# jyjblrd/Low-Cost-Mocap

Measured on AMD Instinct MI355X. Metric: triangulated 3D markers/sec at 8 cams x 16 markers, higher is better.
Workload: dtype f64

## Files before the change

low-cost-mocap_amd/csrc/frame_bb.hip:

```cpp
#include "mocap_device.hpp"
#include "kernels.hpp"
#include <cstdlib>
#include "frame_common.hpp"
#include "bb_fold.hpp"

namespace mocap {

constexpr int kBBThreads = 256;
constexpr int kBBWaves = kBBThreads / 64;
constexpr int kBBRecs = kBBThreads + 64;
constexpr int bb_cw(int C) { return C <= 8 ? 1 : 2; }
constexpr uint32_t bb_rec_bytes(int CW) { return 24u + 8u * (uint32_t)CW; }
constexpr bool bb_group_rows(int CT, int ML, int RL) { return CT > 0 && ML > 0 && RL > 0 && CT * ML < 0xFF && (ML & (ML - 1)) == 0; }

constexpr int bb_wg_per_cu(int RL) { return RL == 48 ? 5 : 4; }
constexpr size_t kBBCacheEntry = 4;
constexpr int kBBLdsSlack = 1024;
struct BBLayout {
  size_t bxy, bxy_nx, cnt_nx, bt, rbound, seedkey, slot_key, claimw, recs, rpk, scr, scr_bytes, goff, gcnt, outslot, boff, bnb, seedgh, slot_g, cnt,
      misc, bpl, nh, hits, act, root_blob, root_cam, nact, bnl, bv, pkbase, seen, bcache, total;
  int ncache;
  __host__ __device__ static size_t al(size_t x, size_t a) { return (x + a - 1) / a * a; }
  __host__ __device__ BBLayout(int C, int M, int R, int CW, int wg_per_cu, bool row_words = false) {
    size_t o = 0;
    auto take = [&](size_t bytes, size_t a) {
      o = al(o, a);
      const size_t at = o;
      o += bytes;
      return at;
    };
    bxy = take(sizeof(float2) * (size_t)C * M, 16);
    bxy_nx = take(sizeof(float2) * (size_t)C * M, 16);
    cnt_nx = take(4 * (size_t)C, 4);
    bt = take(sizeof(double) * 10 * ((size_t)C * M + 1), 16);
    rbound = take(8 * (size_t)R, 8);
    claimw = take(8 * (size_t)C, 8);
    pkbase = take(8 * (size_t)CW * R, 8);
    scr = seedkey = take(8 * (size_t)R, 8);
    slot_key = take(8 * (size_t)kBBWaves * R, 8);
    recs = take(8 * (size_t)kBBRecs, 8);
    rpk = take(8 * (size_t)kBBRecs * CW, 8);
    seedgh = take(4 * (size_t)R, 4);
    slot_g = take(4 * (size_t)kBBWaves * R, 4);
    scr_bytes = o - scr;
    goff = take(4 * (size_t)(R + 1), 4);
    gcnt = take(4 * (size_t)R, 4);
    outslot = take(4 * (size_t)R, 4);
    boff = take(4 * (size_t)(R + 1), 4);
    bnb = take(4 * (size_t)R, 4);
    cnt = take(4 * (size_t)C, 4);
    misc = take(4 * 16, 4);
    bpl = take(2 * (size_t)R, 2);
    seen = take(2 * (size_t)R, 2);
    nh = take((size_t)R * C, row_words ? 8 : 1);
    hits = take((size_t)R * C * M, 1);
    act = take((size_t)R * C, row_words ? 8 : 1);
    root_blob = take((size_t)R, 1);
    root_cam = take((size_t)R, 1);
    nact = take((size_t)R, 1);
    bnl = take((size_t)R, 1);
    bv = take((size_t)R, 1);
    bcache = take(0, 4);
    ncache = 0;
    const size_t per_entry = kBBCacheEntry;
    for (int per_cu = wg_per_cu; per_cu >= 1; per_cu--) {
      const size_t lim = ((size_t)160 * 1024 / per_cu - kBBLdsSlack) / 256 * 256;
      if (lim >= o + per_entry * 64) {
        const size_t n = (lim - o) / per_entry;
        ncache = (int)(n > 1024 ? 1024 : n);
        break;
      }
    }
    o += per_entry * (size_t)ncache;
    total = al(o, 16);
  }
};

static int bb_fixed_slots(int C, int M, int R) {
  const char* e = getenv("MOCAP_BB_FIXED_LAYOUT");
  if (e && e[0] == '0') return 0;
  if (C == 8 && M == 16 && R <= 48) return 48;
  if (C == 8 && M == 16 && R <= 64) return 64;
  return 0;
}
static int frame_bb_root_slots(int C, int M, int R) {
  const int f = bb_fixed_slots(C, M, R);
  return f ? f : R;
}
size_t frame_bb_lds_bytes(int C, int M, int R) { return BBLayout(C, M, frame_bb_root_slots(C, M, R), bb_cw(C), bb_wg_per_cu(bb_fixed_slots(C, M, R)), bb_fixed_slots(C, M, R) != 0).total; }
static size_t frame_bb_lds_bytes_min(int C, int M, int R) {
  const BBLayout L(C, M, frame_bb_root_slots(C, M, R), bb_cw(C), bb_wg_per_cu(bb_fixed_slots(C, M, R)), bb_fixed_slots(C, M, R) != 0);
  return L.total - kBBCacheEntry * (size_t)L.ncache;
}
bool frame_bb_fits(int C, int M, int R) {
  return C >= 2 && C <= 16 && M >= 1 && M <= 64 && R >= 1 && R <= 255 && frame_bb_lds_bytes_min(C, M, R) <= (size_t)128 * 1024;
}

template <int CW, uint32_t NONE = 0xFFu>
struct Packed {
  unsigned long long w[CW];
  __device__ __forceinline__ void clear() {
#pragma unroll
    for (int k = 0; k < CW; k++) w[k] = NONE * 0x0101010101010101ull;
  }
  __device__ __forceinline__ void set(int c, uint32_t idx) {
    if (CW == 1)
      w[0] ^= (unsigned long long)(idx ^ NONE) << (8 * c);
    else
      w[c >> 3] ^= (unsigned long long)(idx ^ NONE) << (8 * (c & 7));
  }
  __device__ __forceinline__ uint32_t get(int c) const {
    return CW == 1 ? (uint32_t)(w[0] >> (8 * c)) & 0xFFu : (uint32_t)(w[c >> 3] >> (8 * (c & 7))) & 0xFFu;
  }
};

template <int CT, bool PERK = false>
struct BBCamTables {
  const double* base;
  static constexpr int C = CT;
  static constexpr int kPq = PERK ? 12 * CT * CT : 12 * CT;
  __device__ __forceinline__ ctab_t pq(size_t off) const { return as_ctab(base + off); }
  __device__ __forceinline__ ctab_t rt(size_t off) const { return as_ctab(base + kPq + off); }
  __device__ __forceinline__ ctab_t k4(size_t off) const { return as_ctab(base + kPq + 12 * CT + off); }
  __device__ __forceinline__ const double* f() const { return base + kPq + 16 * CT; }
};
template <bool PERK>
struct BBCamTables<0, PERK> {
  const double* base;
  int C;
  __device__ __forceinline__ ctab_t pq(size_t off) const { return as_ctab(base + off); }
  __device__ __forceinline__ ctab_t rt(size_t off) const { return as_ctab(base + (PERK ? 12 * C * C : 12 * C) + off); }
  __device__ __forceinline__ ctab_t k4(size_t off) const { return as_ctab(base + (PERK ? 12 * C * C + 12 * C : 24 * C) + off); }
  __device__ __forceinline__ const double* f() const { return base + (PERK ? 12 * C * C + 16 * C : 28 * C); }
};

enum { kPrioEval = 0, kPrioSeed = 1, kPrioPhase = 2, kPrioSerial = 3 };
template <int P>
__device__ __forceinline__ void bb_prio() {
  __builtin_amdgcn_s_setprio(P);
}

__device__ __forceinline__ float f32_round_up(double v) {
  const float f = (float)v;
  const int32_t b = __float_as_int(f);
  return (double)f < v ? __int_as_float(b + ((b >> 31) | 1)) : f;
}

template <bool F32R, int CW, int CT, int ML, int RL, bool PERK = false>
struct BBState {
  static constexpr int T = kBBThreads, W = kBBWaves;
  static constexpr bool ROWS = bb_group_rows(CT, ML, RL);
  static constexpr uint32_t kNone = ROWS ? (uint32_t)(CT * ML) : 0xFFu;
  typedef Packed<CW, kNone> Pk;
  static_assert(!ROWS || (CT == 8 && CW == 1), "a row of nh / act as one word: eight cameras");
  __device__ __forceinline__ unsigned long long row_word64(const uint8_t* rows, int r) const { return ((const unsigned long long*)rows)[r]; }
  __device__ static __forceinline__ uint32_t byte_of(unsigned long long w, uint32_t k) { return (uint32_t)(w >> (8u * k)) & 0xFFu; }
  static constexpr bool PLIST = CT > 0 && ML > 0 && RL > 0 && ML < 32 && CT * ML <= 256 && (ML & (ML - 1)) == 0;
  __device__ __forceinline__ uint32_t gbyte(int c, uint32_t k) const { return ROWS ? (uint32_t)c * (uint32_t)ML + k : k; }
  __device__ __forceinline__ size_t grow(int c, uint32_t b) const { return ROWS ? (size_t)b : (size_t)c * M + b; }
  const FrameArgs& p;
  BBCamTables<CT, PERK> cv;
  const int C_, M, R, RS;
  int tid, lane, wave;
  __device__ __forceinline__ void fresh_tid() {
    int t = tid;
    asm volatile("" : "+v"(t));
    tid = t;
    lane = t & 63;
    wave = t >> 6;
  }
  __device__ __forceinline__ int cn() const { return CT > 0 ? CT : C_; }
  enum { PC_OTHER = 0, PC_PAIRS0, PC_PAIRS1, PC_B1_TABLE, PC_ROW_COPY, PC_PHASE_C, PC_SEED_PASS, PC_SEED_PUSH, PC_EVAL, PC_TEST, PC_PHASE_E, PC_COUNT };
#ifdef MOCAP_BB_PHASE_CLOCKS
  uint32_t pc_last = 0, pc_sum[PC_COUNT] = {};
  template <int PH>
  __device__ __forceinline__ void pc_mark() {
    if (__builtin_amdgcn_readfirstlane((int)threadIdx.x >> 6) == 0) {
      const uint32_t now = (uint32_t)__builtin_readcyclecounter();
      pc_sum[PH] += now - pc_last;
      pc_last = now;
    }
  }
  __device__ __forceinline__ void pc_start() { pc_last = (uint32_t)__builtin_readcyclecounter(); }
  __device__ __forceinline__ void pc_flush() const {
    if (threadIdx.x == 0 && !p.n_frames_dev)
      for (int k = 0; k < PC_COUNT; k++) atomicAdd(&p.status[p.n_frames + k], (int)(pc_sum[k] >> 8));
  }
#else
  template <int PH>
  __device__ __forceinline__ void pc_mark() {}
  __device__ __forceinline__ void pc_start() {}
  __device__ __forceinline__ void pc_flush() const {}
#endif
  double* bt;
  float2 *bxy, *bxy_nx;
  int32_t* cnt_nx;
  unsigned long long *rbound, *seedkey, *slot_key, *claimw, *rpk;
  struct BRec { uint32_t gh, rs; };
  BRec* recs;
  uint32_t *goff, *gcnt, *boff, *bnb, *seedgh, *slot_g;
  int32_t *outslot, *cnt, *misc;
  uint16_t* bpl;
  uint8_t *nh, *hits, *act, *root_blob, *root_cam, *nact, *bnl, *bv;
  float* bcache;
  unsigned long long* pkbase;
  uint16_t* seen;
  int ncache;
  unsigned char* scr;
  size_t scr_bytes;
  static constexpr unsigned long long kInfBits = 0x7ff0000000000000ull;

  __device__ BBState(const FrameArgs& p_, unsigned char* smem)
      : p(p_), C_(p_.cv.C), M(ML > 0 ? ML : p_.M), R(p_.K_max), RS(RL > 0 ? RL : p_.K_max), tid(threadIdx.x), lane(threadIdx.x & 63), wave(threadIdx.x >> 6) {
    const int C = cn();
    {
      const unsigned long long ta = (unsigned long long)(uintptr_t)p_.cv.Pq;
      uint32_t tlo = (uint32_t)__builtin_amdgcn_readfirstlane((int)(uint32_t)ta);
      uint32_t thi = (uint32_t)__builtin_amdgcn_readfirstlane((int)(uint32_t)(ta >> 32));
      asm volatile("" : "+s"(tlo), "+s"(thi));
      cv.base = (const double*)(uintptr_t)(((unsigned long long)thi << 32) | tlo);
      if constexpr (CT == 0) cv.C = C;
    }
    const BBLayout L(C, M, RS, CW, bb_wg_per_cu(RL), ROWS);
    bt = (double*)(smem + L.bt);
    bxy = (float2*)(smem + L.bxy);
    bxy_nx = (float2*)(smem + L.bxy_nx);
    cnt_nx = (int32_t*)(smem + L.cnt_nx);
    rbound = (unsigned long long*)(smem + L.rbound);
    seedkey = (unsigned long long*)(smem + L.seedkey);
    slot_key = (unsigned long long*)(smem + L.slot_key);
    claimw = (unsigned long long*)(smem + L.claimw);
    recs = (BRec*)(smem + L.recs);
    rpk = (unsigned long long*)(smem + L.rpk);
    goff = (uint32_t*)(smem + L.goff);
    gcnt = (uint32_t*)(smem + L.gcnt);
    outslot = (int32_t*)(smem + L.outslot);
    boff = (uint32_t*)(smem + L.boff);
    bnb = (uint32_t*)(smem + L.bnb);
    seedgh = (uint32_t*)(smem + L.seedgh);
    slot_g = (uint32_t*)(smem + L.slot_g);
    cnt = (int32_t*)(smem + L.cnt);
    misc = (int32_t*)(smem + L.misc);
    bpl = (uint16_t*)(smem + L.bpl);
    nh = (uint8_t*)(smem + L.nh);
    hits = (uint8_t*)(smem + L.hits);
    act = (uint8_t*)(smem + L.act);
    root_blob = (uint8_t*)(smem + L.root_blob);
    root_cam = (uint8_t*)(smem + L.root_cam);
    nact = (uint8_t*)(smem + L.nact);
    bnl = (uint8_t*)(smem + L.bnl);
    bv = (uint8_t*)(smem + L.bv);
    scr = smem + L.scr;
    scr_bytes = L.scr_bytes;
    bcache = (float*)(smem + L.bcache);
    pkbase = (unsigned long long*)(smem + L.pkbase);
    seen = (uint16_t*)(smem + L.seen);
    ncache = L.ncache;
  }

  struct Line { double a, b, c, den, rden; };
  __device__ __forceinline__ Line epiline(int r, int i) const { return epiline_of(root_cam[r], root_blob[r], i); }
  __device__ __forceinline__ Line epiline_of(int rc, int rb, int i) const {
    const int C = cn();
    const double* Fm = cv.f() + 9 * ((size_t)rc * C + i);
    const float2 rp = bxy[(size_t)rc * M + rb];
    const double x = (double)rp.x, y = (double)rp.y;
    double a = Fm[0] * x + Fm[1] * y + Fm[2];
    double b = Fm[3] * x + Fm[4] * y + Fm[5];
    double c = Fm[6] * x + Fm[7] * y + Fm[8];
    double nu = a * a + b * b;
    nu = nu != 0.0 ? 1.0 / sqrt(nu) : 1.0;
    a *= nu;
    b *= nu;
    c *= nu;
    if (F32R) {
      a = (double)(float)a;
      b = (double)(float)b;
      c = (double)(float)c;
    }
    Line L;
    L.a = a;
    L.b = b;
    L.c = c;
    L.den = sqrt(a * a + b * b);
    L.rden = recip_refined(L.den);
    return L;
  }

  template <bool CHAIN>
  __device__ __forceinline__ unsigned long long match_pairs(const Line& mine, int pair_r, int pair_i, int n_pairs, int gs_shift,
                                                            int cam = 0, int Mi_chain = 0) {
    const int C = cn();
    const int GS = 1 << gs_shift, PPS = 64 >> gs_shift;
    const int k = lane & (GS - 1), q = lane >> gs_shift;
    const int gl0 = lane & ~(GS - 1);
    const unsigned long long gall = gs_shift == 6 ? ~0ull : ((1ull << GS) - 1ull);
    unsigned long long claims = 0ull;
    for (int s0 = 0; s0 < n_pairs; s0 += PPS) {
      const int src = s0 + q;
      const bool has = src < n_pairs;
      const int sl = has ? src : 0;
      const double la = __shfl(mine.a, sl), lb = __shfl(mine.b, sl), lc = __shfl(mine.c, sl);
      const double lden = __shfl(mine.den, sl), lrden = __shfl(mine.rden, sl);
      const int r = __shfl(pair_r, sl);
      const int i = CHAIN ? cam : __shfl(pair_i, sl);
      const int Mi = has ? (CHAIN ? Mi_chain : cnt[i]) : 0;
      const bool valid = k < Mi;
      float2 pt = make_float2(0.f, 0.f);
      double d = 0.0;
      bool hit = false;
      if (valid) {
        pt = bxy[(size_t)i * M + k];
        const double num = fabs(la * (double)pt.x + lb * (double)pt.y + lc);
        d = div_by(num, lden, lrden);
        hit = d < p.gate_px;
      }
      const unsigned long long wm = __ballot(hit);
      const unsigned long long gm = (wm >> gl0) & gall;
      int rank = 0;
      const unsigned int dlo = (unsigned int)__double_as_longlong(d), dhi = (unsigned int)(__double_as_longlong(d) >> 32);
      for (unsigned long long mm = wm; mm;) {
        const int j = __ffsll((long long)mm) - 1;
        mm &= mm - 1;
        const double dj = __longlong_as_double(((long long)__builtin_amdgcn_readlane((int)dhi, j) << 32) |
                                               (unsigned int)__builtin_amdgcn_readlane((int)dlo, j));
        const bool mine_grp = (j & ~(GS - 1)) == gl0 && j != lane;
        rank += (hit && mine_grp && (dj < d || (dj == d && j < lane))) ? 1 : 0;
      }
      if (hit) hits[((size_t)r * C + i) * M + rank] = (uint8_t)gbyte(i, (uint32_t)k);
      const unsigned long long g0 = (__ballot(hit && rank == 0) >> gl0) & gall;
      bool same = false;
      if (valid && g0) {
        const float2 p0 = bxy[(size_t)i * M + (__ffsll((long long)g0) - 1)];
        same = pt.x == p0.x && pt.y == p0.y;
      }
      const unsigned long long cw = __ballot(same);
      if (CHAIN) {
        for (int sh = 0; sh < 64; sh += GS) claims |= (cw >> sh) & gall;
      }
      if (has && k == 0) {
        nh[(size_t)r * C + i] = (uint8_t)__popcll(gm);
        if (!CHAIN) {
          const unsigned long long cm = (cw >> gl0) & gall;
          if (cm) atomicOr(&claimw[i], cm);
        }
      }
    }
    return claims;
  }

  __device__ __forceinline__ void prefetch_lds(int64_t frame) const {
    const int C = cn();
    const float* src = p.blobs + (size_t)frame * C * M * 2;
    const int n_dw = C * M * 2;
    for (int base = wave * 64; base < n_dw; base += T)
      if (base + lane < n_dw)
        __builtin_amdgcn_global_load_lds((const __attribute__((address_space(1))) void*)(src + base + lane),
                                         (__attribute__((address_space(3))) void*)((float*)bxy_nx + base), 4, 0, 0);
    if (wave == 0 && lane < C)
      __builtin_amdgcn_global_load_lds((const __attribute__((address_space(1))) void*)(p.counts + (size_t)frame * C + lane),
                                       (__attribute__((address_space(3))) void*)cnt_nx, 4, 0, 0);
  }
  __device__ __forceinline__ void stage(int64_t frame) {
    fresh_tid();
    const int C = cn();
    float2* t = bxy;
    bxy = bxy_nx;
    bxy_nx = t;
    if (tid < C) {
      const int n = cnt_nx[tid];
      cnt[tid] = n < 0 ? 0 : (n > M ? M : n);
      claimw[tid] = 0ull;
    }
    if (tid == 0) {
      misc[MI_STATUS] = 0;
      misc[MI_OMAX] = 0;
    }
  }

  __device__ void match() {
    fresh_tid();
    const int C = cn();
    __syncthreads();
    int gs_shift = 0;
    while ((1 << gs_shift) < M) gs_shift++;
    const int n0 = cnt[0] < R ? cnt[0] : R;
    {
      for (int r = tid; r < n0; r += T) {
        root_cam[r] = 0;
        root_blob[r] = (uint8_t)r;
      }
      if (tid == 0 && cnt[0] > R) misc[MI_STATUS] |= MOCAP_ST_ROOT_OVERFLOW_;
    }
    __syncthreads();
    auto U_of = [&](int j) {
      const int n = cnt[j];
      return ~claimw[j] & (n >= 64 ? ~0ull : ((1ull << n) - 1ull));
    };
    int n_prov = 0, n_ppairs = 0;
    bool pre = false;
    uint8_t* nh_s = nullptr;
    uint8_t* hits_s = nullptr;
    unsigned long long* pclaim = (unsigned long long*)scr;
    uint8_t* plist = act;
    uint32_t* p_end = goff;
    {
      int Mmax = 0;
      for (int c = 1; c < C; c++) Mmax = cnt[c] > Mmax ? cnt[c] : Mmax;
#pragma nounroll
      for (int stage_ = 0; stage_ < 2; stage_++) {
        const int stage = __builtin_amdgcn_readfirstlane(stage_);
        int NP = n0 * (C - 1);
        if (stage == 1) {
          block_sync_lds();
          pc_mark<PC_PAIRS0>();
          if constexpr (PLIST) {
#pragma unroll
            for (int j = 1; j < CT; j++) {
              const uint32_t U = ~((const uint32_t*)claimw)[2 * j] & ((1u << cnt[j]) - 1u);
              if (lane < ML && ((U >> lane) & 1u)) plist[__builtin_amdgcn_mbcnt_lo(U, (uint32_t)n_prov)] = (uint8_t)(j * ML + lane);
              n_prov += __popc(U);
              n_ppairs += __popc(U) * (CT - 1 - j);
              if (lane == 0) p_end[j] = ((uint32_t)n_ppairs << 16) | (uint32_t)n_prov;
            }
            wave_lds_sync();
          } else
          for (int j = 1; j < C; j++) {
            const int np = __popcll(U_of(j));
            n_prov += np;
            n_ppairs += np * (C - 1 - j);
          }
          pre = n_prov <= 64 && (size_t)n_prov * C * (8 + 1 + (size_t)M) <= scr_bytes;
          if (!pre) break;
          nh_s = (uint8_t*)(pclaim + (size_t)n_prov * C);
          hits_s = nh_s + (size_t)n_prov * C;
          NP = n_ppairs;
        }
        for (int base = wave * 64; base < NP; base += W * 64) {
          const int pi = base + lane;
          const bool have = pi < NP;
          int r = 0, i = 1, Mi = 0;
          Line L = {0, 0, 0, 1, 1};
          if (have) {
            if (stage == 0) {
              r = pi / (C - 1);
              i = 1 + (pi - r * (C - 1));
              L = epiline(r, i);
            } else if constexpr (PLIST) {
              int j = 1;
              uint32_t before = 0;
              const uint32_t key = ((uint32_t)pi << 16) | 0xFFFFu;
              uint32_t pe[CT > 2 ? CT - 2 : 1];
#pragma unroll
              for (int jj = 1; jj <= CT - 2; jj++) pe[jj - 1] = p_end[jj];
#pragma unroll
              for (int jj = 1; jj <= CT - 2; jj++) {
                const bool ge = key >= pe[jj - 1];
                j += ge ? 1 : 0;
                before = ge ? pe[jj - 1] : before;
              }
              const uint32_t acc = before >> 16, pb = before & 0xFFFFu;
              uint32_t ord, off;
              divmod_tiny((uint32_t)pi - acc, (uint32_t)(CT - 1 - j), ord, off);
              r = (int)(pb + ord);
              const int k = plist[r] & (ML - 1);
              i = j + 1 + (int)off;
              L = epiline_of(j, k, i);
            } else {
              int j = 1, acc = 0, pb = 0, span = C - 2;
              unsigned long long U = 0ull;
              for (; j <= C - 2; j++) {
                span = C - 1 - j;
                U = U_of(j);
                const int nj = __popcll(U) * span;
                if (pi < acc + nj) break;
                acc += nj;
                pb += __popcll(U);
              }
              uint32_t ord, off;
              divmod_tiny((uint32_t)(pi - acc), (uint32_t)span, ord, off);
              for (uint32_t t = 0; t < ord; t++) U &= U - 1;
              const int k = __ffsll((long long)U) - 1;
              i = j + 1 + (int)off;
              r = pb + (int)ord;
              L = epiline_of(j, k, i);
            }
            Mi = cnt[i];
          }
          const float2* pts = bxy + (size_t)i * M;
          auto dist = [&](int k) {
            const float2 pt = pts[k];
            return div_by(fabs(L.a * (double)pt.x + L.b * (double)pt.y + L.c), L.den, L.rden);
          };
          unsigned long long hm = 0ull;
          double bd0 = __builtin_huge_val();
          int bk0 = 0;
          if constexpr (ROWS) {
            static_assert(ML % 2 == 0 && ML < 32, "two blobs per word, the slots as bits of one register");
            const float4* pw = (const float4*)pts;
            uint32_t cand = (1u << Mi) - 1u;
            uint32_t hw = 0u;
            if constexpr (F32R) {
              static_assert(CT * ML == 128, "the frame's slots: one word of two blobs per lane");
              uint32_t ob;
              {
                const float4 v = ((const float4*)bxy)[lane];
                const int n = cnt[lane / (ML / 2)], k0 = 2 * (lane % (ML / 2));
                const uint32_t ax = __float_as_uint(v.x) & 0x7FFFFFFFu, ay = __float_as_uint(v.y) & 0x7FFFFFFFu;
                const uint32_t az = __float_as_uint(v.z) & 0x7FFFFFFFu, aw = __float_as_uint(v.w) & 0x7FFFFFFFu;
                const uint32_t m0 = k0 < n ? (ax > ay ? ax : ay) : 0u, m1 = k0 + 1 < n ? (az > aw ? az : aw) : 0u;
                ob = m0 > m1 ? m0 : m1;
                auto up = [](uint32_t x, uint32_t y) { return x > y ? x : y; };
                ob = up(ob, (uint32_t)__builtin_amdgcn_update_dpp(0, (int)ob, 0xB1, 0xf, 0xf, true));
                ob = up(ob, (uint32_t)__builtin_amdgcn_update_dpp(0, (int)ob, 0x4E, 0xf, 0xf, true));
                ob = up(ob, (uint32_t)__builtin_amdgcn_update_dpp(0, (int)ob, 0x141, 0xf, 0xf, true));
                ob = up(ob, (uint32_t)__builtin_amdgcn_update_dpp(0, (int)ob, 0x140, 0xf, 0xf, true));
                const uint32_t r0 = (uint32_t)__builtin_amdgcn_readlane((int)ob, 0), r1 = (uint32_t)__builtin_amdgcn_readlane((int)ob, 16);
                const uint32_t r2 = (uint32_t)__builtin_amdgcn_readlane((int)ob, 32), r3 = (uint32_t)__builtin_amdgcn_readlane((int)ob, 48);
                ob = up(up(r0, r1), up(r2, r3));
                ob = ob < 0x7F800000u ? ob : 0x7F800000u;
              }
              const double om = (double)__uint_as_float(ob);
              const float a32 = (float)L.a, b32 = (float)L.b, c32 = (float)L.c;
              const float thr = f32_round_up(p.gate_px * L.den * (1.0 + 1e-12) + (2.5 * 0x1p-24) * (2.0 * om + fabs(L.c)) * (1.0 + 1e-6));
              uint32_t pm = 0u;
#pragma unroll
              for (int h = ML / 2 - 1; h >= 0; h--) {
                const float4 v = pw[h];
                float t0 = fmaf(a32, v.x, fmaf(b32, v.y, c32)), t1 = fmaf(a32, v.z, fmaf(b32, v.w, c32));
                asm("" : "+v"(t0), "+v"(t1));
                pm = pm + pm + (fabsf(t1) <= thr ? 1u : 0u);
                pm = pm + pm + (fabsf(t0) <= thr ? 1u : 0u);
              }
              cand &= pm;
              while (__ballot(cand != 0u)) {
                if (cand) {
                  const int k = __ffs((int)cand) - 1;
                  cand &= cand - 1u;
                  const double d = dist(k);
                  if (d < p.gate_px) {
                    hw |= 1u << k;
                    if (d < bd0) {
                      bd0 = d;
                      bk0 = k;
                    }
                  }
                }
              }
            } else {
#pragma unroll
              for (int h = 0; h < ML / 2; h++) {
                const float4 v = pw[h];
                const double d0 = div_by(fabs(L.a * (double)v.x + L.b * (double)v.y + L.c), L.den, L.rden);
                const double d1 = div_by(fabs(L.a * (double)v.z + L.b * (double)v.w + L.c), L.den, L.rden);
                const bool h0 = d0 < p.gate_px && ((cand >> (2 * h)) & 1u), h1 = d1 < p.gate_px && ((cand >> (2 * h + 1)) & 1u);
                hw |= h0 ? 1u << (2 * h) : 0u;
                const bool b0 = h0 && d0 < bd0;
                bd0 = b0 ? d0 : bd0;
                bk0 = b0 ? 2 * h : bk0;
                hw |= h1 ? 2u << (2 * h) : 0u;
                const bool b1 = h1 && d1 < bd0;
                bd0 = b1 ? d1 : bd0;
                bk0 = b1 ? 2 * h + 1 : bk0;
              }
            }
            hm = hw;
          } else
#pragma unroll 4
          for (int k = 0; k < Mmax; k++)
            if (k < Mi && dist(k) < p.gate_px) hm |= 1ull << k;
          uint8_t* nhp = stage == 0 ? nh : nh_s;
          uint8_t* hl = (stage == 0 ? hits : hits_s) + ((size_t)r * C + i) * M;
          if (have) nhp[(size_t)r * C + i] = (uint8_t)__popcll(hm);
          unsigned long long rem = hm, claim = 0ull;
          int pos = 0;
          float2 p0 = make_float2(0.f, 0.f);
          if constexpr (ROWS) {
            if (hm) {
              hl[0] = (uint8_t)gbyte(i, (uint32_t)bk0);
              claim = hm;
              if (hm & (hm - 1ull)) {
                claim = 0ull;
                p0 = pts[bk0];
                for (unsigned long long t = hm; t; t &= t - 1) {
                  const int k = __ffsll((long long)t) - 1;
                  const float2 q = pts[k];
                  if (q.x == p0.x && q.y == p0.y) claim |= 1ull << k;
                }
              }
              rem = hm & ~(1ull << bk0);
              pos = 1;
            }
          }
          while (__ballot(rem != 0ull)) {
            if (rem) {
              double bd = __builtin_huge_val();
              int bk = 0;
              if (ROWS && !(rem & (rem - 1ull))) {
                bk = __ffsll((long long)rem) - 1;
              } else
              for (unsigned long long t = rem; t; t &= t - 1) {
                const int k = __ffsll((long long)t) - 1;
                const double d = dist(k);
                if (d < bd) {
                  bd = d;
                  bk = k;
                }
              }
              hl[pos] = (uint8_t)gbyte(i, (uint32_t)bk);
              if (!ROWS && pos == 0) {
                p0 = pts[bk];
                for (unsigned long long t = hm; t; t &= t - 1) {
                  const int k = __ffsll((long long)t) - 1;
                  const float2 q = pts[k];
                  if (q.x == p0.x && q.y == p0.y) claim |= 1ull << k;
                }
              }
              rem &= ~(1ull << bk);
              pos++;
            }
          }
          if (stage == 0) {
            if (claim) atomicOr(&claimw[i], claim);
          } else if (have) {
            pclaim[(size_t)r * C + i] = claim;
          }
        }
      }
    }
    const int NL = M * ((C - 1) * (C - 2) / 2);
    const bool spec = F32R && (size_t)NL * 20 + 8 <= scr_bytes;
    double* sp_den = (double*)scr;
    float* sp_abc = (float*)(sp_den + NL);
    auto sp_base = [&](int j) { return M * ((j - 1) * (C - 1) - (j - 1) * j / 2); };
    if (spec && !pre) {
      int tot = 0;
      for (int j = 1; j <= C - 2; j++) {
        const int n = cnt[j];
        const unsigned long long U = ~claimw[j] & (n >= 64 ? ~0ull : ((1ull << n) - 1ull));
        tot += __popcll(U) * (C - 1 - j);
      }
      for (int l = tid; l < tot; l += T) {
        int j = 1, acc = 0, span = C - 2;
        unsigned long long U = 0ull;
        for (; j <= C - 2; j++) {
          const int n = cnt[j];
          U = ~claimw[j] & (n >= 64 ? ~0ull : ((1ull << n) - 1ull));
          span = C - 1 - j;
          const int nj = __popcll(U) * span;
          if (l < acc + nj) break;
          acc += nj;
        }
        uint32_t ord, off;
        divmod_tiny((uint32_t)(l - acc), (uint32_t)span, ord, off);
        for (uint32_t t = 0; t < ord; t++) U &= U - 1;
        const int k = __ffsll((long long)U) - 1, i = j + 1 + (int)off;
        const int ll = sp_base(j) + k * span + (int)off;
        const Line L = epiline_of(j, k, i);
        sp_den[ll] = L.den;
        sp_abc[3 * ll + 0] = (float)L.a;
        sp_abc[3 * ll + 1] = (float)L.b;
        sp_abc[3 * ll + 2] = (float)L.c;
      }
    }
    __syncthreads();
    pc_mark<PC_PAIRS1>();
    fresh_tid();
    if (wave == 0) bb_prio<kPrioSerial>();
    if (wave == 0 && pre) {
      int jp = 0, kp = 0;
      if constexpr (PLIST) {
        if (lane < n_prov) {
          const int row = plist[lane];
          jp = row / ML;
          kp = row & (ML - 1);
        }
      } else
      if (lane < n_prov) {
        int acc = 0;
        unsigned long long U = 0ull;
        for (jp = 1; jp < C; jp++) {
          U = U_of(jp);
          const int np = __popcll(U);
          if (lane < acc + np) break;
          acc += np;
        }
        for (int t = 0; t < lane - acc; t++) U &= U - 1;
        kp = __ffsll((long long)U) - 1;
      }
      bool real = false;
      for (int i = 1; i < C; i++) {
        wave_lds_sync();
        if (lane < n_prov && jp == i) {
          real = !((claimw[i] >> kp) & 1ull);
          if (real)
            for (int c = i + 1; c < C; c++) {
              const unsigned long long m = pclaim[(size_t)lane * C + c];
              if (m) atomicOr(&claimw[c], m);
            }
        }
      }
      const unsigned long long rm = __ballot(real);
      const int rank = __popcll(rm & ((1ull << lane) - 1ull));
      int n_roots = n0 + __popcll(rm);
      if (real && n0 + rank < R) {
        root_cam[n0 + rank] = (uint8_t)jp;
        root_blob[n0 + rank] = (uint8_t)kp;
        bnl[rank] = (uint8_t)lane;
      }
      if (lane == 0) {
        if (n_roots > R) {
          misc[MI_STATUS] |= MOCAP_ST_ROOT_OVERFLOW_;
          n_roots = R;
        }
        misc[MI_NROOTS] = n_roots;
      }
    } else if (wave == 0) {
      const int cntL = lane < C ? cnt[lane] : 0;
      const unsigned long long clmL = lane < C ? claimw[lane] : 0ull;
      int nr_cam = 0, nr_blob = 0;
      int n_roots = n0;
      bool over = false;
      for (int i = 1; i < C; i++) {
        const int Mi = __builtin_amdgcn_readlane(cntL, i);
        unsigned long long claimed = ((unsigned long long)(unsigned int)__builtin_amdgcn_readlane((int)(clmL >> 32), i) << 32) |
                                     (unsigned int)__builtin_amdgcn_readlane((int)clmL, i);
        const int n_new = n_roots - n0;
        for (int base = 0; base < n_new; base += 64) {
          const int l = base + lane;
          const bool have = l < n_new;
          int j = nr_cam, k = nr_blob;
          if (base) {
            wave_lds_sync();
            j = have ? root_cam[n0 + l] : 0;
            k = have ? root_blob[n0 + l] : 0;
          }
          Line L = {0, 0, 0, 1, 1};
          if (have) {
            if (spec) {
              const int ll = sp_base(j) + k * (C - 1 - j) + (i - j - 1);
              L.a = (double)sp_abc[3 * ll + 0];
              L.b = (double)sp_abc[3 * ll + 1];
              L.c = (double)sp_abc[3 * ll + 2];
              L.den = sp_den[ll];
              L.rden = recip_refined(L.den);
            } else {
              L = epiline_of(j, k, i);
            }
          }
          claimed |= match_pairs<true>(L, n0 + l, i, (n_new - base < 64) ? n_new - base : 64, gs_shift, i, Mi);
        }
        const bool flag = lane < Mi && !((claimed >> lane) & 1ull);
        const unsigned long long mask = __ballot(flag);
        const int pos = __popcll(mask & ((1ull << lane) - 1ull));
        if (flag) {
          const int rr = n_roots + pos;
          if (rr < R) {
            root_cam[rr] = (uint8_t)i;
            root_blob[rr] = (uint8_t)lane;
          }
        }
        int slot = n_new;
        for (unsigned long long mm = mask; mm; slot++) {
          const int jb = __ffsll((long long)mm) - 1;
          mm &= mm - 1;
          if (lane == slot) {
            nr_cam = i;
            nr_blob = jb;
          }
        }
        n_roots += __popcll(mask);
        if (n_roots > R) {
          over = true;
          n_roots = R;
        }
      }
      if (lane == 0) {
        if (over) misc[MI_STATUS] |= MOCAP_ST_ROOT_OVERFLOW_;
        misc[MI_NROOTS] = n_roots;
      }
    } else {
      float om = 0.0f;
      for (int i = tid - 64; i < C * M; i += T - 64) {
        const int c = i / M, k = i - c * M;
        if (k < cnt[c]) {
          const float2 v = bxy[i];
          om = fmaxf(om, fmaxf(fabsf(v.x), fabsf(v.y)));
          double Bc[10];
          dlt_contribution(Bc, cv.pq(PERK ? 12 * (c * C + c) : 12 * c), (double)v.x, (double)v.y);
#pragma unroll
          for (int e = 0; e < 10; e++) bt[(size_t)i * 10 + e] = Bc[e];
        }
      }
      if (om > 0.0f) atomicMax(&misc[MI_OMAX], __float_as_int(om));
      if (tid == 64) {
        const int it = q_add(&p.q.counters[QC_NEXT_FRAME], 1);
        misc[MI_NEXT] = it < frame_count(p) ? it : -1;
      }
    }
    bb_prio<kPrioPhase>();
    __syncthreads();
    pc_mark<PC_B1_TABLE>();
    if (pre) {
      const int n_new = misc[MI_NROOTS] - n0;
      for (int idx = tid; idx < n_new * C; idx += T) {
        const int q = idx / C, c = idx - q * C;
        const int r = n0 + q, ps = bnl[q];
        if (c > (int)root_cam[r]) {
          const int n = nh_s[(size_t)ps * C + c];
          nh[(size_t)r * C + c] = (uint8_t)n;
          const uint8_t* src = hits_s + ((size_t)ps * C + c) * M;
          uint8_t* dst = hits + ((size_t)r * C + c) * M;
          for (int t = 0; t < n; t++) dst[t] = src[t];
        }
      }
      __syncthreads();
      pc_mark<PC_ROW_COPY>();
    }

    fresh_tid();
    const int nroots = misc[MI_NROOTS];
    for (int r = tid; r < nroots; r += T) {
      if constexpr (ROWS) {
        const uint32_t rc = root_cam[r], rb = root_blob[r];
        unsigned long long nw = row_word64(nh, r);
        const uint8_t* hr = hits + (size_t)r * (CT * ML);
        uint32_t h1[CT];
#pragma unroll
        for (int c = 1; c < CT; c++) h1[c] = hr[c * ML];
        nw &= (~0ull << (8u * rc)) << 8;
        Pk pkb;
        pkb.clear();
        pkb.set((int)rc, gbyte((int)rc, rb));
        static_assert(CT <= 8 && ML <= 16, "a digit's byte: three bits of camera, four of hit count - 1");
        unsigned long long ew = 0ull;
        uint32_t total = 1, views = 1, na = 0, sm = 1u << rc;
#pragma unroll
        for (int c = CT - 1; c >= 1; c--) {
          const uint32_t n = byte_of(nw, (uint32_t)c);
          if (n > 1) {
            ew = (ew << 8) | (unsigned long long)((n << 3) + (uint32_t)(c - 8));
            na++;
          }
          if (n == 1) pkb.set(c, h1[c]);
          if (n) {
            sm |= 1u << c;
            views++;
            total *= n;
          }
        }
        const unsigned long long aw = ew & 0x0707070707070707ull;
        const unsigned long long dn = ((ew >> 3) & 0x0F0F0F0F0F0F0F0Full) + 0x0101010101010101ull;
        const bool over = (unsigned long long)total > (unsigned long long)p.G_cap;
        if (over) atomicOr(&misc[MI_STATUS], MOCAP_ST_CAND_OVERFLOW_);
        ((unsigned long long*)act)[r] = aw;
        nact[r] = (uint8_t)na;
        bv[r] = (uint8_t)views;
        pkbase[r] = pkb.w[0];
        if (PERK) seen[r] = (uint16_t)sm;
        rbound[r] = kInfBits;
        const uint32_t g = (views > 1 && !over) ? total : 0u;
        gcnt[r] = g;
        uint32_t pl = 1, nb = over ? 1u : total;
        uint32_t nl = 0;
        while (nl < na && (pl < (uint32_t)p.bb_pl_min || (pl < (uint32_t)p.bb_pl && nb > (uint32_t)p.bb_nb_max))) {
          const uint32_t n = byte_of(dn, nl++);
          uint32_t dummy;
          pl *= n;
          divmod_small(nb, n, nb, dummy);
        }
        bpl[r] = (uint16_t)pl;
        bnl[r] = (uint8_t)nl;
        bnb[r] = g ? nb : 0u;
        seedkey[r] = 0ull;
        seedgh[r] = 0xFFFFFFFFu;
        continue;
      }
      const int rc = root_cam[r];
      unsigned long long total = 1;
      int views = 1, na = 0;
      bool over = false;
      Pk pkb;
      pkb.clear();
      pkb.set(rc, gbyte(rc, root_blob[r]));
      uint32_t sm = 1u << rc;
      for (int c = rc + 1; c < C; c++) {
        const unsigned n = nh[(size_t)r * C + c];
        if (n > 1) act[(size_t)r * C + na++] = (uint8_t)c;
        if (n == 1) pkb.set(c, hits[((size_t)r * C + c) * M]);
        if (n) {
          sm |= 1u << c;
          views++;
          total *= n;
          if (total > (unsigned long long)p.G_cap) {
            over = true;
            total = 1;
          }
        }
      }
      if (over) atomicOr(&misc[MI_STATUS], MOCAP_ST_CAND_OVERFLOW_);
      nact[r] = (uint8_t)na;
      bv[r] = (uint8_t)views;
#pragma unroll
      for (int k = 0; k < CW; k++) pkbase[(size_t)r * CW + k] = pkb.w[k];
      if (PERK) seen[r] = (uint16_t)sm;
      rbound[r] = kInfBits;
      const uint32_t g = (views > 1 && !over) ? (uint32_t)total : 0u;
      gcnt[r] = g;
      {
        const uint8_t* a = act + (size_t)r * C;
        uint32_t pl = 1, nb = 1;
        int nl = 0;
        for (int k = 0; k < na; k++) nb *= nh[(size_t)r * C + a[k]];
        if (over) nb = 1;
        while (nl < na && (pl < (uint32_t)p.bb_pl_min || (pl < (uint32_t)p.bb_pl && nb > (uint32_t)p.bb_nb_max))) {
          const uint32_t n = nh[(size_t)r * C + a[nl++]];
          uint32_t dummy;
          pl *= n;
          divmod_small(nb, n, nb, dummy);
        }
        bpl[r] = (uint16_t)pl;
        bnl[r] = (uint8_t)nl;
        bnb[r] = g ? nb : 0u;
// ... 566 lines not shown
```

Baseline: 667.9 million.

## Keep top hits in registers and emit sorted hit list via rank network

Hoists the per-frame coordinate max reduction out of the per-pair loop and makes the candidate scan branchless. It also tracks up to four gated hits per pair in registers. When every lane has at most four hits, it writes the distance-ordered hit bytes as one 32-bit word using a pairwise rank network and computes the claim mask directly. This replaces the repeated argmin-selection loop, cutting serial divergent work, at the cost of extra registers and an extra code path. Ties are handled by index order, which may differ from the selection loop's.

```diff
diff --git a/low-cost-mocap_amd/csrc/frame_bb.hip b/low-cost-mocap_amd/csrc/frame_bb.hip
--- a/low-cost-mocap_amd/csrc/frame_bb.hip
+++ b/low-cost-mocap_amd/csrc/frame_bb.hip
@@ -3,6 +3,7 @@
 #include <cstdlib>
 #include "frame_common.hpp"
 #include "bb_fold.hpp"
+#include "pair_order.hpp"
 
 namespace mocap {
 
@@ -407,6 +408,29 @@
     {
       int Mmax = 0;
       for (int c = 1; c < C; c++) Mmax = cnt[c] > Mmax ? cnt[c] : Mmax;
+      uint32_t omax_bits = 0u;
+      if constexpr (ROWS && F32R) {
+        static_assert(CT * ML == 128, "the frame's slots: one word of two blobs per lane");
+        uint32_t ob;
+        {
+          const float4 v = ((const float4*)bxy)[lane];
+          const int n = cnt[lane / (ML / 2)], k0 = 2 * (lane % (ML / 2));
+          const uint32_t ax = __float_as_uint(v.x) & 0x7FFFFFFFu, ay = __float_as_uint(v.y) & 0x7FFFFFFFu;
+          const uint32_t az = __float_as_uint(v.z) & 0x7FFFFFFFu, aw = __float_as_uint(v.w) & 0x7FFFFFFFu;
+          const uint32_t m0 = k0 < n ? (ax > ay ? ax : ay) : 0u, m1 = k0 + 1 < n ? (az > aw ? az : aw) : 0u;
+          ob = m0 > m1 ? m0 : m1;
+          auto up = [](uint32_t x, uint32_t y) { return x > y ? x : y; };
+          ob = up(ob, (uint32_t)__builtin_amdgcn_update_dpp(0, (int)ob, 0xB1, 0xf, 0xf, true));
+          ob = up(ob, (uint32_t)__builtin_amdgcn_update_dpp(0, (int)ob, 0x4E, 0xf, 0xf, true));
+          ob = up(ob, (uint32_t)__builtin_amdgcn_update_dpp(0, (int)ob, 0x141, 0xf, 0xf, true));
+          ob = up(ob, (uint32_t)__builtin_amdgcn_update_dpp(0, (int)ob, 0x140, 0xf, 0xf, true));
+          const uint32_t r0 = (uint32_t)__builtin_amdgcn_readlane((int)ob, 0), r1 = (uint32_t)__builtin_amdgcn_readlane((int)ob, 16);
+          const uint32_t r2 = (uint32_t)__builtin_amdgcn_readlane((int)ob, 32), r3 = (uint32_t)__builtin_amdgcn_readlane((int)ob, 48);
+          ob = up(up(r0, r1), up(r2, r3));
+          ob = ob < 0x7F800000u ? ob : 0x7F800000u;
+        }
+        omax_bits = ob;
+      }
 #pragma nounroll
       for (int stage_ = 0; stage_ < 2; stage_++) {
         const int stage = __builtin_amdgcn_readfirstlane(stage_);
@@ -442,30 +466,40 @@
           int r = 0, i = 1, Mi = 0;
           Line L = {0, 0, 0, 1, 1};
           if (have) {
-            if (stage == 0) {
+            if constexpr (PLIST) {
+              static_assert(PLIST == ROWS, "the listed provisional roots and the table rows: the same layouts");
+              int rc, rb;
+              if (stage == 0) {
+                r = pi / (C - 1);
+                i = 1 + (pi - r * (C - 1));
+                rc = root_cam[r];
+                rb = root_blob[r];
+              } else {
+                int j = 1;
+                uint32_t before = 0;
+                const uint32_t key = ((uint32_t)pi << 16) | 0xFFFFu;
+                uint32_t pe[CT > 2 ? CT - 2 : 1];
+#pragma unroll
+                for (int jj = 1; jj <= CT - 2; jj++) pe[jj - 1] = p_end[jj];
+#pragma unroll
+                for (int jj = 1; jj <= CT - 2; jj++) {
+                  const bool ge = key >= pe[jj - 1];
+                  j += ge ? 1 : 0;
+                  before = ge ? pe[jj - 1] : before;
+                }
+                const uint32_t acc = before >> 16, pb = before & 0xFFFFu;
+                uint32_t ord, off;
+                divmod_tiny((uint32_t)pi - acc, (uint32_t)(CT - 1 - j), ord, off);
+                r = (int)(pb + ord);
+                rc = j;
+                rb = plist[r] & (ML - 1);
+                i = j + 1 + (int)off;
+              }
+              L = epiline_of(rc, rb, i);
+            } else if (stage == 0) {
               r = pi / (C - 1);
               i = 1 + (pi - r * (C - 1));
               L = epiline(r, i);
-            } else if constexpr (PLIST) {
-              int j = 1;
-              uint32_t before = 0;
-              const uint32_t key = ((uint32_t)pi << 16) | 0xFFFFu;
-              uint32_t pe[CT > 2 ? CT - 2 : 1];
-#pragma unroll
-              for (int jj = 1; jj <= CT - 2; jj++) pe[jj - 1] = p_end[jj];
-#pragma unroll
-              for (int jj = 1; jj <= CT - 2; jj++) {
-                const bool ge = key >= pe[jj - 1];
-                j += ge ? 1 : 0;
-                before = ge ? pe[jj - 1] : before;
-              }
-              const uint32_t acc = before >> 16, pb = before & 0xFFFFu;
-              uint32_t ord, off;
-              divmod_tiny((uint32_t)pi - acc, (uint32_t)(CT - 1 - j), ord, off);
-              r = (int)(pb + ord);
-              const int k = plist[r] & (ML - 1);
-              i = j + 1 + (int)off;
-              L = epiline_of(j, k, i);
             } else {
               int j = 1, acc = 0, pb = 0, span = C - 2;
               unsigned long long U = 0ull;
@@ -495,32 +529,18 @@
           unsigned long long hm = 0ull;
           double bd0 = __builtin_huge_val();
           int bk0 = 0;
+          constexpr bool KEPT = ROWS && F32R;
+          constexpr int NK = 4;
+          double kd[NK];
+          uint32_t kk[NK];
+          if constexpr (KEPT) pair_keep_init<NK>(kd, kk);
           if constexpr (ROWS) {
             static_assert(ML % 2 == 0 && ML < 32, "two blobs per word, the slots as bits of one register");
             const float4* pw = (const float4*)pts;
             uint32_t cand = (1u << Mi) - 1u;
             uint32_t hw = 0u;
             if constexpr (F32R) {
-              static_assert(CT * ML == 128, "the frame's slots: one word of two blobs per lane");
-              uint32_t ob;
-              {
-                const float4 v = ((const float4*)bxy)[lane];
-                const int n = cnt[lane / (ML / 2)], k0 = 2 * (lane % (ML / 2));
-                const uint32_t ax = __float_as_uint(v.x) & 0x7FFFFFFFu, ay = __float_as_uint(v.y) & 0x7FFFFFFFu;
-                const uint32_t az = __float_as_uint(v.z) & 0x7FFFFFFFu, aw = __float_as_uint(v.w) & 0x7FFFFFFFu;
-                const uint32_t m0 = k0 < n ? (ax > ay ? ax : ay) : 0u, m1 = k0 + 1 < n ? (az > aw ? az : aw) : 0u;
-                ob = m0 > m1 ? m0 : m1;
-                auto up = [](uint32_t x, uint32_t y) { return x > y ? x : y; };
-                ob = up(ob, (uint32_t)__builtin_amdgcn_update_dpp(0, (int)ob, 0xB1, 0xf, 0xf, true));
-                ob = up(ob, (uint32_t)__builtin_amdgcn_update_dpp(0, (int)ob, 0x4E, 0xf, 0xf, true));
-                ob = up(ob, (uint32_t)__builtin_amdgcn_update_dpp(0, (int)ob, 0x141, 0xf, 0xf, true));
-                ob = up(ob, (uint32_t)__builtin_amdgcn_update_dpp(0, (int)ob, 0x140, 0xf, 0xf, true));
-                const uint32_t r0 = (uint32_t)__builtin_amdgcn_readlane((int)ob, 0), r1 = (uint32_t)__builtin_amdgcn_readlane((int)ob, 16);
-                const uint32_t r2 = (uint32_t)__builtin_amdgcn_readlane((int)ob, 32), r3 = (uint32_t)__builtin_amdgcn_readlane((int)ob, 48);
-                ob = up(up(r0, r1), up(r2, r3));
-                ob = ob < 0x7F800000u ? ob : 0x7F800000u;
-              }
-              const double om = (double)__uint_as_float(ob);
+              const double om = (double)__uint_as_float(omax_bits);
               const float a32 = (float)L.a, b32 = (float)L.b, c32 = (float)L.c;
               const float thr = f32_round_up(p.gate_px * L.den * (1.0 + 1e-12) + (2.5 * 0x1p-24) * (2.0 * om + fabs(L.c)) * (1.0 + 1e-6));
               uint32_t pm = 0u;
@@ -534,18 +554,16 @@
               }
               cand &= pm;
               while (__ballot(cand != 0u)) {
-                if (cand) {
-                  const int k = __ffs((int)cand) - 1;
-                  cand &= cand - 1u;
-                  const double d = dist(k);
-                  if (d < p.gate_px) {
-                    hw |= 1u << k;
-                    if (d < bd0) {
-                      bd0 = d;
-                      bk0 = k;
-                    }
-                  }
-                }
+                const bool live = cand != 0u;
+                const int k = (__ffs((int)cand) - 1) & (ML - 1);
+                cand &= cand - 1u;
+                const double d = dist(k);
+                const bool h = live && d < p.gate_px;
+                hw |= h ? 1u << k : 0u;
+                pair_keep<NK>(kd, kk, h, d, (uint32_t)k);
+                const bool b = h && d < bd0;
+                bd0 = b ? d : bd0;
+                bk0 = b ? k : bk0;
               }
             } else {
 #pragma unroll
@@ -575,6 +593,25 @@
           unsigned long long rem = hm, claim = 0ull;
           int pos = 0;
           float2 p0 = make_float2(0.f, 0.f);
+          bool kept = false;
+          if constexpr (KEPT) {
+            kept = __ballot(__popc((uint32_t)hm) > NK) == 0ull;
+            if (kept && hm) {
+              uint32_t kg[NK];
+              float qx[NK], qy[NK];
+              p0 = pts[bk0];
+#pragma unroll
+              for (int a = 0; a < NK; a++) {
+                kg[a] = gbyte(i, kk[a]);
+                const float2 q = pts[kk[a]];
+                qx[a] = q.x;
+                qy[a] = q.y;
+              }
+              *(uint32_t*)hl = pair_order_word<NK>(kd, kg);
+              claim = (unsigned long long)(pair_claim_mask<NK>(p0.x, p0.y, qx, qy, kk) & (uint32_t)hm);
+            }
+          }
+          if (!KEPT || !kept) {
           if constexpr (ROWS) {
             if (hm) {
               hl[0] = (uint8_t)gbyte(i, (uint32_t)bk0);
@@ -619,6 +656,7 @@
               rem &= ~(1ull << bk);
               pos++;
             }
+          }
           }
           if (stage == 0) {
             if (claim) atomicOr(&claimw[i], claim);
diff --git a/low-cost-mocap_amd/csrc/pair_order.hpp b/low-cost-mocap_amd/csrc/pair_order.hpp
--- /dev/null
+++ b/low-cost-mocap_amd/csrc/pair_order.hpp
@@ -0,0 +1,64 @@
+#pragma once
+#include <cstdint>
+
+#if defined(__HIPCC__) || defined(__CUDACC__)
+#define PAIR_ORDER_HD __host__ __device__ __forceinline__
+#else
+#define PAIR_ORDER_HD inline
+#endif
+
+template <int NK>
+PAIR_ORDER_HD void pair_keep_init(double (&d)[NK], uint32_t (&k)[NK]) {
+#pragma unroll
+  for (int a = 0; a < NK; a++) {
+    d[a] = __builtin_huge_val();
+    k[a] = 0u;
+  }
+}
+
+template <int NK>
+PAIR_ORDER_HD void pair_keep(double (&d)[NK], uint32_t (&k)[NK], bool hit, double dn, uint32_t kn) {
+#pragma unroll
+  for (int a = NK - 1; a > 0; a--) {
+    d[a] = hit ? d[a - 1] : d[a];
+    k[a] = hit ? k[a - 1] : k[a];
+  }
+  d[0] = hit ? dn : d[0];
+  k[0] = hit ? kn : k[0];
+}
+
+PAIR_ORDER_HD bool pair_precedes(double da, double db) {
+#ifdef MOCAP_PAIR_ORDER_TIES_BY_LATER
+  return da <= db;
+#else
+  return da < db;
+#endif
+}
+
+template <int NK>
+PAIR_ORDER_HD uint32_t pair_order_word(const double (&d)[NK], const uint32_t (&g)[NK]) {
+  static_assert(NK >= 1 && NK <= 4, "the ordered list is one 32-bit word");
+  uint32_t sh[NK];
+#pragma unroll
+  for (int a = 0; a < NK; a++) sh[a] = 8u * (uint32_t)(NK - 1 - a);
+#pragma unroll
+  for (int a = 0; a < NK; a++)
+#pragma unroll
+    for (int b = a + 1; b < NK; b++) {
+      const uint32_t c = pair_precedes(d[a], d[b]) ? 8u : 0u;
+      sh[b] += c;
+      sh[a] -= c;
+    }
+  uint32_t w = 0u;
+#pragma unroll
+  for (int a = 0; a < NK; a++) w |= g[a] << sh[a];
+  return w;
+}
+
+template <int NK>
+PAIR_ORDER_HD uint32_t pair_claim_mask(float p0x, float p0y, const float (&qx)[NK], const float (&qy)[NK], const uint32_t (&k)[NK]) {
+  uint32_t m = 0u;
+#pragma unroll
+  for (int a = 0; a < NK; a++) m |= (qx[a] == p0x && qy[a] == p0y) ? 1u << k[a] : 0u;
+  return m;
+}
```

New measurement: 673.4 million, median of 6. Within noise of the previous version (+0.8%).
